# 30stomercury/whisper-char-alignment

Hardware: AMD Instinct MI355X
Metric: utterances/sec (whisper-medium, 10s audio, char align) at 1/2/4/8 MI355X (higher is better)
Workload: dtype f16x2 (hi + lo operand pairs on the f16 MFMA pipe: fp32-equivalent operands, fp32 accumulate)

## Files before the change

### whisper-char-alignment_amd/csrc/engine.hip

```cpp
#include <hip/hip_runtime.h>
#include <dlfcn.h>
#include <rccl/rccl.h>

#include <chrono>
#include <cmath>
#include <cstdarg>
#include <cstdio>
#include <cstdlib>
#include <cstring>
#include <deque>
#include <map>
#include <set>
#include <string>
#include <vector>

#include "../../include/wca.h"
#include "kernels.h"

using namespace wca;

namespace {

thread_local std::string g_err;

// ... 2877 lines not shown

int wca_test_gemm(wca_engine* e, const void* a, const void* w, const float* bias, void* c, int M, int N, int K, int gelu, int out_mode) {
  if (!e) return fail(WCA_ERR_INVALID, "null engine");
  HIPCHK(hipSetDevice(e->device));
  GemmArgs g{};
  g.A = (const half_t*)a;
  g.lda = K;
  g.W = (const half_t*)w;
  g.ldw = K;
  g.bias = bias;
  g.C = c;
  g.ldc = N;
  g.M = M;
  g.N = N;
  g.K = K;
  g.gelu = gelu;
  g.out_mode = out_mode & 0xff;
  if (g.out_mode == 4) {
    g.ldc = 2 * N;
    g.c_lo = N;
  }
  g.force_tile = (out_mode >> 8) & 0xfff;
  g.supertile = out_mode >> 20;
  g.sk_part = e->sk_big[0];
  g.sk_bytes = e->sk_big_bytes;
  HIPCHK(launch_gemm(g, e->stream));
  return WCA_OK;
}

int wca_test_gemm_pairs(wca_engine* e, const void* a2, const void* w, const float* bias, void* c, int M, int N, int K, int gelu, int out_mode) {
  if (!e || !a2 || !w || !c) return fail(WCA_ERR_INVALID, "null argument");
  HIPCHK(hipSetDevice(e->device));
  const int om = out_mode & 0xff;
  if (!gemm_splitw_supported(M, N, K, 2 * K, om)) return fail(WCA_ERR_INVALID, "the pair-operand kernel does not take M=%d N=%d K=%d out_mode %d", M, N, K, om);
  GemmArgs g{};
  g.A = (const half_t*)a2;
  g.lda = 2 * K;
  g.a_lo = K;
  g.W = (const half_t*)w;
  g.ldw = K;
  g.bias = bias;
  g.C = c;
  g.ldc = N;
  g.M = M;
  g.N = N;
  g.K = K;
  g.gelu = gelu;
  g.out_mode = om;
  if (om == 4) {
    g.ldc = 2 * N;
    g.c_lo = N;
  }
  g.force_tile = (out_mode >> 8) & 0xfff;
  g.site = 1;
  HIPCHK(launch_gemm(g, e->stream));
  return WCA_OK;
}

int wca_test_gemm_ln(wca_engine* e, const void* a, const void* w, const float* bias, float* x, const float* gamma, const float* beta,
                     void* xn, int M, int N, int K, int site) {
  if (!e || !a || !w || !x || !gamma || !beta || !xn) return fail(WCA_ERR_INVALID, "null argument");
  HIPCHK(hipSetDevice(e->device));
  if (!gemm_ln_supported(M, N, K, e->n_cu)) return fail(WCA_ERR_INVALID, "residual + LayerNorm epilogue not available for M=%d N=%d K=%d", M, N, K);
  const size_t mpad = align_up((size_t)M, 256);
  HIPCHK(e->tmp0.ensure(sizeof(unsigned long long) * (size_t)(N / 256) * mpad));
  HIPCHK(e->tmp1.ensure(sizeof(unsigned) * (mpad / 256 + 16)));
  HIPCHK(hipMemsetAsync(e->err_dev, 0, sizeof(int), e->stream));
// ... 236 lines not shown
```

### whisper-char-alignment_amd/csrc/gemm.hip

```cpp
#include <atomic>

#include "gemm_epilogue.h"
#include <cstdlib>
#include "kernels.h"
#include "wca_common.h"

namespace wca {

namespace {

constexpr int BM = 128, BN = 128, BK = 64;
constexpr int TILE_ELEMS = 128 * 64;

struct RowPtrs {
  const half_t* p[4];
};

__device__ __forceinline__ half8 ldfrag(const half_t* tile, int r, int c) {
  return *reinterpret_cast<const half8*>(tile + r * 64 + ((c ^ swz128(r)) << 3));
}

template <int OUT_MODE, bool GELU, int MT>
__device__ __forceinline__ void epilogue(const GemmArgs& a, f32x4 (&acc)[MT][4], int mbase, int nb, int fr) {
  float bv[16];
// ... 318 lines not shown
      for (int mt = 0; mt < 4; ++mt)
#pragma unroll
        for (int nt = 0; nt < 4; ++nt)
          acc[mt][nt] = __builtin_amdgcn_mfma_f32_16x16x32_f16(wf[ks][nt], xf[ks][mt], acc[mt][nt], 0, 0, 0);
    __builtin_amdgcn_s_setprio(0);

    half8 xg[2][4];
#pragma unroll
    for (int ks = 0; ks < 2; ++ks)
#pragma unroll
      for (int t = 0; t < 4; ++t) xg[ks][t] = ldfrag(At, xrow[4 + t], ks * 4 + fg);
    asm volatile("s_waitcnt lgkmcnt(0)" ::: "memory");
    __builtin_amdgcn_s_barrier();
    asm volatile("" ::: "memory");
    if (kt + 2 < nk) stage(cur, (kt + 2) * BK);
    __builtin_amdgcn_s_setprio(1);
#pragma unroll
    for (int ks = 0; ks < 2; ++ks)
#pragma unroll
      for (int mt = 0; mt < 4; ++mt)
#pragma unroll
        for (int nt = 0; nt < 4; ++nt)
          acc[4 + mt][nt] = __builtin_amdgcn_mfma_f32_16x16x32_f16(wf[ks][nt], xg[ks][mt], acc[4 + mt][nt], 0, 0, 0);
    __builtin_amdgcn_s_setprio(0);
  }

  epilogue<OUT_MODE, GELU, 8>(a, acc, m0 + wr * 128, n0 + wc * 64 + fg * 16, fr);
}

template <int V>
struct GemmIntC {
  static constexpr int value = V;
};

template <int OUT_MODE, bool GELU, int SITE, int SPLITW_MODE = 0>
__global__ __launch_bounds__(512) void gemm256p_f16_kernel(GemmArgs a) {
  constexpr bool SPLITW = SPLITW_MODE != 0;
  constexpr bool RING3 = SPLITW_MODE == 2;
  extern __shared__ __attribute__((aligned(16))) char smem[];
  half_t* lds = reinterpret_cast<half_t*>(smem);
  constexpr int TILE256 = 256 * 64;
  float* bias_lds = reinterpret_cast<float*>(smem + 4 * TILE256 * sizeof(half_t));
  float* gamma_lds = bias_lds + 512;
  float* beta_lds = gamma_lds + 512;
  float* ln_lds = beta_lds + 512;
  const int tid = threadIdx.x;
  const int lane = tid & 63;
  const int wave = __builtin_amdgcn_readfirstlane(tid >> 6);
  const int wr = wave >> 2, wc = wave & 3;

  const int ntn = (a.N + 255) / 256;
  const int ntm = (a.M + 255) / 256;
  const int nwg = ntm * ntn;
  const int G = gridDim.x;

  const __amdgpu_buffer_rsrc_t ra = __builtin_amdgcn_make_buffer_rsrc(const_cast<half_t*>(a.A), 0, (int)a.a_bytes, 0x00020000);
  const __amdgpu_buffer_rsrc_t rw = __builtin_amdgcn_make_buffer_rsrc(const_cast<half_t*>(a.W), 0, (int)a.w_bytes, 0x00020000);
  const __amdgpu_buffer_rsrc_t rb = __builtin_amdgcn_make_buffer_rsrc(const_cast<float*>(a.bias), 0, a.bias != nullptr ? a.N * 4 : 0, 0x00020000);
  const __amdgpu_buffer_rsrc_t rg = __builtin_amdgcn_make_buffer_rsrc(const_cast<float*>(a.ln_gamma), 0, OUT_MODE == 3 ? a.N * 4 : 0, 0x00020000);
  const __amdgpu_buffer_rsrc_t rbeta = __builtin_amdgcn_make_buffer_rsrc(const_cast<float*>(a.ln_beta), 0, OUT_MODE == 3 ? a.N * 4 : 0, 0x00020000);
  const int l8 = lane >> 3;
  const int rho = wave * 8 + l8;
  const int c0 = (lane & 7) ^ ((rho >> 1) & 7);
  const int nt_r = rho >> 4, i_r = rho & 15;
  const int wsrc_row = (OUT_MODE == 0 || OUT_MODE == 3 || OUT_MODE == 4) ? ((nt_r >> 1) * 32 + (i_r >> 2) * 8 + (nt_r & 1) * 4 + (i_r & 3)) : rho;
  const unsigned va = (unsigned)(rho * a.lda + c0 * 8) * 2u;
// ... 17 lines not shown
  auto stage_bias = [&](int par, int ncol0) {
    if (wave < 4) {
      __builtin_amdgcn_raw_ptr_buffer_load_lds(rb, (WCA_LDS void*)(bias_lds + par * 256 + wave * 64), 4, (ncol0 + wave * 64 + lane) * 4, 0, 0, 0);
      if (OUT_MODE == 3) {
        __builtin_amdgcn_raw_ptr_buffer_load_lds(rg, (WCA_LDS void*)(gamma_lds + par * 256 + wave * 64), 4, (ncol0 + wave * 64 + lane) * 4, 0, 0, 0);
        __builtin_amdgcn_raw_ptr_buffer_load_lds(rbeta, (WCA_LDS void*)(beta_lds + par * 256 + wave * 64), 4, (ncol0 + wave * 64 + lane) * 4, 0, 0, 0);
      }
    }
  };
  constexpr int RING3_A_REQS_IN_FLIGHT = 4;
  static_assert(RING3_A_REQS_IN_FLIGHT * 64 == 256, "one request per 64-row block of the 256-row A tile");

  const int fr = lane & 15, fg = lane >> 4;
  const int pos0 = fg ^ ((fr >> 1) & 7);
  const int xb0 = (wr * 128 + fr) * 64 + pos0 * 8, xb1 = (wr * 128 + fr) * 64 + (pos0 ^ 4) * 8;
  const int wb0 = (wc * 64 + fr) * 64 + pos0 * 8, wb1 = (wc * 64 + fr) * 64 + (pos0 ^ 4) * 8;

#define WCA_LOAD_HALF(AT, WT, XB, WB, WF, XF)                                                      \
  do {                                                                                             \
    _Pragma("unroll") for (int t = 0; t < 4; ++t) WF[t] = *reinterpret_cast<const half8*>((WT) + (WB) + t * 1024); \
    _Pragma("unroll") for (int t = 0; t < 8; ++t) XF[t] = *reinterpret_cast<const half8*>((AT) + (XB) + t * 1024); \
  } while (0)

  const int nk = SPLITW ? 2 * (a.K / BK) : a.K / BK;
  auto a_koff = [&](int s_) -> unsigned {
    return SPLITW ? (unsigned)(((s_ & 1) * (int)a.a_lo + (s_ >> 1) * BK) * 2) : (unsigned)(s_ * (BK * 2));
  };
  auto w_koff = [&](int s_) -> unsigned {
    return SPLITW ? (unsigned)((s_ >> 1) * (BK * 2)) : (unsigned)(s_ * (BK * 2));
  };
  int v = blockIdx.x;
  int id = xcd_remap(v, nwg);
  const int SM = a.supertile > 0 ? a.supertile : 1;
  auto tile_of = [&](int t, int& tm, int& tn) {
    const int per = SM * ntn;
    const int st = t / per, r = t - st * per;
    const int rows = (ntm - st * SM) < SM ? (ntm - st * SM) : SM;
    tn = r / rows;
    tm = st * SM + (r - tn * rows);
  };
  const int spx = G >> 3;
  const int PR = spx / ntn;
  const int lab = blockIdx.x & 7, slot = blockIdx.x >> 3;
  const int pq = ntm >> 3, prm = ntm & 7;
  const int lab_panels = pq + (lab < prm ? 1 : 0), lab_base = lab * pq + (lab < prm ? lab : prm);
  auto tile_of_round = [&](int round, int& tm, int& tn) -> bool {
    tn = slot / PR;
    const int pi = round * PR + (slot - tn * PR);
    tm = lab_base + pi;
    return tn < ntn && pi < lab_panels;
  };
  int tm_, tn_;
  int round = 0;
  if (OUT_MODE == 3) {
    if (!tile_of_round(0, tm_, tn_)) return;
  } else {
    tile_of(id, tm_, tn_);
  }
  int m0 = tm_ * 256, n0 = tn_ * 256;
  unsigned ta = (unsigned)m0 * a.lda * 2u, tw = (unsigned)n0 * a.ldw * 2u;

  f32x4 acc[8][4];
#pragma unroll
  for (int i = 0; i < 8; ++i)
#pragma unroll
    for (int j = 0; j < 4; ++j) acc[i][j] = f32x4{0.f, 0.f, 0.f, 0.f};
  half8 w0[4], x0[8], w1[4], x1[8];
  int par = 0;
  stage_bias(0, n0);
#pragma unroll
  for (int g = 0; g < 8; ++g) stage_one(0, 0, ta, tw, g);
  if (nk > 1) {
#pragma unroll
// ... 99 lines not shown

    {
      int fr_e = fr, fg_e = fg;
      asm volatile("" : "+v"(fr_e), "+v"(fg_e));
      typedef __attribute__((address_space(4))) GemmArgs KernArgs;
      const KernArgs* ap = (const KernArgs*)__builtin_amdgcn_kernarg_segment_ptr();
      asm volatile("" : "+s"(ap));
      if constexpr (OUT_MODE == 3)
        epilogue_ln<KernArgs>(*ap, acc, m0, m0 >> 8, n0 >> 8, ntn, wr, wc, fr_e, fg_e, bias_lds + par * 256 + wc * 64, gamma_lds + par * 256,
                              beta_lds + par * 256, ln_lds);
      else
        epilogue_wide<OUT_MODE, GELU, KernArgs>(*ap, acc, m0 + wr * 128, n0 + wc * 64, fr_e, fg_e, bias_lds + par * 256 + wc * 64);
    }
    if (!has_next) break;
    par ^= 1;
    stage_bias(par, n0n);
    v = vn;
    id = idn;
    ++round;
    m0 = m0n;
    n0 = n0n;
    ta = tan;
    tw = twn;
#pragma unroll
    for (int i = 0; i < 8; ++i)
#pragma unroll
      for (int j = 0; j < 4; ++j) acc[i][j] = f32x4{0.f, 0.f, 0.f, 0.f};
    WCA_LOAD_HALF(a_slot(RING3 ? ring_a : 0), w_slot(0), xb0, wb0, w0, x0);
  }
#undef WCA_LOAD_HALF
}


template <int OUT_MODE, bool GELU>
__global__ __launch_bounds__(256) void gemm_skinny_f16_kernel(GemmArgs a) {
  __shared__ float red[4][4][4][64];
  const int tid = threadIdx.x;
  const int lane = tid & 63;
  const int wave = __builtin_amdgcn_readfirstlane(tid >> 6);
  const int fr = lane & 15, fg = lane >> 4;
  const int n0 = blockIdx.x * 16;
  const int kq = a.K >> 2;
  const int kbeg = wave * kq;
  int nrow = n0 + fr;
  nrow = nrow < a.N ? nrow : a.N - 1;
  const half_t* wp = a.W + (long)nrow * a.ldw + kbeg + fg * 8;
  const half_t* xp[4];
#pragma unroll
  for (int mt = 0; mt < 4; ++mt) {
    int m = mt * 16 + fr;
    m = m < a.M ? m : a.M - 1;
    xp[mt] = a.A + (long)m * a.lda + kbeg + fg * 8;
  }
  f32x4 acc[4];
#pragma unroll
  for (int mt = 0; mt < 4; ++mt) acc[mt] = f32x4{0.f, 0.f, 0.f, 0.f};
  half8 wf[2][4], xf[2][4][4];
  auto load_chunk = [&](int buf, int k) {
#pragma unroll
    for (int u = 0; u < 4; ++u) {
      wf[buf][u] = *reinterpret_cast<const half8*>(wp + k + u * 32);
#pragma unroll
      for (int mt = 0; mt < 4; ++mt) xf[buf][u][mt] = *reinterpret_cast<const half8*>(xp[mt] + k + u * 32);
    }
  };
  auto mul_chunk = [&](int buf) {
// ... 37 lines not shown
    half_t* cp = reinterpret_cast<half_t*>(a.C) + coff + nb;
    if (nb + 4 <= a.N && (reinterpret_cast<uintptr_t>(cp) & 7) == 0) {
      half4 o;
#pragma unroll
      for (int r = 0; r < 4; ++r) o[r] = (half_t)v[r];
      *reinterpret_cast<half4*>(cp) = o;
    } else {
#pragma unroll
      for (int r = 0; r < 4; ++r)
        if (nb + r < a.N) cp[r] = (half_t)v[r];
    }
  } else {
    float* cp = reinterpret_cast<float*>(a.C) + coff + nb;
#pragma unroll
    for (int r = 0; r < 4; ++r)
      if (nb + r < a.N) cp[r] = (OUT_MODE == 2) ? cp[r] + v[r] : v[r];
  }
}

}

bool gemm_ln_supported(int M, int N, int K, int n_cu) {
  if (N % 256 != 0 || N > 2048 || K % 128 != 0 || M < 1) return false;
  const long tiles = (long)((M + 255) / 256) * (N / 256);
  if (tiles < 192) return false;
  return (n_cu >> 3) >= N / 256;
}

bool gemm_splitw_supported(int M, int N, int K, int lda, int out_mode) {
  if (M < 1 || N < 1 || K < 128 || (K % 128) != 0) return false;
  if (out_mode != 0 && out_mode != 1 && out_mode != 2 && out_mode != 4) return false;
  const long tiles256 = (long)((M + 255) / 256) * ((N + 255) / 256);
  if (tiles256 < 192) return false;
  const size_t a_need = ((size_t)(M - 1) * lda + 2 * (size_t)K) * sizeof(half_t), w_need = ((size_t)(N - 1) * K + K) * sizeof(half_t);
  return a_need < 0x7fffffffull && w_need < 0x7fffffffull;
}

hipError_t launch_gemm(const GemmArgs& a_in, hipStream_t s) {
  GemmArgs a = a_in;
  if (a.M <= 0 || a.N <= 0) return hipSuccess;
  if (a.K <= 0 || (a.K % BK) != 0) return hipErrorInvalidValue;
  if ((a.lda % 8) != 0 || (a.ldw % 8) != 0) return hipErrorInvalidValue;
  if (a.out_mode == 4 && (a.c_lo <= 0 || (a.c_lo & 7))) return hipErrorInvalidValue;
  if (a.addend != nullptr && (a.out_mode == 2 || a.out_mode == 3 || a.a_lo > 0)) return hipErrorInvalidValue;
  if ((a.force_tile == 64 || a.force_tile == 0) && a.M <= 64 && (a.K % 512) == 0 && a.a_rows_per_batch == 0 && a.pos == nullptr && a.addend == nullptr && a.out_mode != 4 && a.a_lo <= 0) {
    const dim3 sgrid((unsigned)((a.N + 15) / 16)), sblock(256);
#define WCA_LAUNCH_SK(OM, G) hipLaunchKernelGGL((gemm_skinny_f16_kernel<OM, G>), sgrid, sblock, 0, s, a)
    if (a.out_mode == 0) {
      if (a.gelu) WCA_LAUNCH_SK(0, true); else WCA_LAUNCH_SK(0, false);
    } else if (a.out_mode == 1) {
      if (a.gelu) WCA_LAUNCH_SK(1, true); else WCA_LAUNCH_SK(1, false);
    } else if (a.out_mode == 2 && !a.gelu) {
      WCA_LAUNCH_SK(2, false);
    } else {
      return hipErrorInvalidValue;
    }
#undef WCA_LAUNCH_SK
    return hipGetLastError();
  }
  if (a.force_tile == 64) return hipErrorInvalidValue;
  const long tiles256 = (long)((a.M + 255) / 256) * ((a.N + 255) / 256);
  const bool splitw = a.a_lo > 0;
  if (splitw && (a.force_tile == 64 || a.force_tile == 128 || a.force_tile == 256 || a.a_rows_per_batch != 0 ||
                 !gemm_splitw_supported(a.M, a.N, a.K, a.lda, a.out_mode) || (a.a_lo & 7) != 0))
    return hipErrorInvalidValue;
  const size_t a_need = ((size_t)(a.M - 1) * a.lda + (splitw ? (size_t)a.a_lo : 0) + a.K) * sizeof(half_t), w_need = ((size_t)(a.N - 1) * a.ldw + a.K) * sizeof(half_t);
  const bool can_buf = a.a_rows_per_batch == 0 && a_need < 0x7fffffffull && w_need < 0x7fffffffull;
  if (a.a_bytes == 0) a.a_bytes = (unsigned)a_need;
  if (a.w_bytes == 0) a.w_bytes = (unsigned)w_need;
  int dev = 0;
  {
    hipError_t e = hipGetDevice(&dev);
    if (e != hipSuccess) return e;
  }
  static std::atomic<int> n_cu_cache[32] = {};
  int n_cu = n_cu_cache[dev & 31].load(std::memory_order_relaxed);
  if (n_cu == 0) {
    hipError_t e = hipDeviceGetAttribute(&n_cu, hipDeviceAttributeMultiprocessorCount, dev);
    if (e != hipSuccess) return e;
    n_cu_cache[dev & 31].store(n_cu, std::memory_order_relaxed);
  }
  if (a.cu_limit > 0 && a.cu_limit < n_cu) n_cu = a.cu_limit;
  const int ring = splitw ? (debug_switch(DBG_GEMM_RING) == 1 ? 1 : 2) : 0;
  const bool want_big = (a.force_tile == 256 || a.force_tile == 257 || a.force_tile == 258) || (a.force_tile == 0 && tiles256 >= 192);
  const bool pipelined = want_big && can_buf && a.force_tile != 256 && a.addend == nullptr;
  const bool big = want_big;
  dim3 grid, block;
  size_t shmem;
  int splitk = 1;
  if (big) {
    grid = dim3((unsigned)tiles256);
    block = dim3(512);
    shmem = 2 * 2 * 256 * 64 * sizeof(half_t);
    if (pipelined) {
      shmem += 2 * 256 * sizeof(float);
      const int nk = (splitw ? 2 : 1) * (a.K / BK);
      if (a.force_tile != 258 && nk >= 2 && (nk & 1) == 0 && tiles256 > n_cu) grid = dim3((unsigned)n_cu);
      if (a.supertile <= 0) a.supertile = ((splitw ? 2 : 1) * a.K <= 2048 && (a.N + 255) / 256 <= 32) ? 8 : 1;
    }
  } else {
    const int ntn = (a.N + BN - 1) / BN, ntm = (a.M + BM - 1) / BM;
    grid = dim3(ntn * ntm);
    block = dim3(256);
    shmem = 2 * 2 * TILE_ELEMS * sizeof(half_t);
    splitk = 1;
    if (a.out_mode == 2 && !a.gelu && a.sk_part != nullptr && a.pos == nullptr && a.c_rows_per_batch == 0 && (a.N % 4) == 0 && (a.ldc % 4) == 0 &&
        ntn * ntm <= n_cu / 2 && a.K >= 2048) {
      for (int sk = 4; sk >= 2; --sk)
        if (a.K % (sk * BK) == 0 && (size_t)sk * a.M * a.N * sizeof(float) <= a.sk_bytes) {
          splitk = sk;
          break;
        }
    }
    grid.y = (unsigned)splitk;
  }
#define WCA_LAUNCH_K(...)                                                                         \
  do {                                                                                            \
    static std::atomic<unsigned> attr_mask{0};                                                    \
    if (!(attr_mask.load(std::memory_order_acquire) & (1u << (dev & 31)))) {                      \
      hipError_t e = hipFuncSetAttribute(reinterpret_cast<const void*>(__VA_ARGS__),              \
                                         hipFuncAttributeMaxDynamicSharedMemorySize, (int)shmem); \
      if (e != hipSuccess) return e;                                                              \
      attr_mask.fetch_or(1u << (dev & 31), std::memory_order_release);                            \
    }                                                                                             \
    hipLaunchKernelGGL((__VA_ARGS__), grid, block, shmem, s, a);                                  \
  } while (0)
#define WCA_LAUNCH_S(OM, G, S)                            \
  do {                                                    \
    if (pipelined && splitw && ring == 1) { if ((S) == 4) WCA_LAUNCH_K(gemm256p_f16_kernel<OM, G, 4, 1>); else WCA_LAUNCH_K(gemm256p_f16_kernel<OM, G, 1, 1>); } \
    else if (pipelined && splitw) { if ((S) == 4) WCA_LAUNCH_K(gemm256p_f16_kernel<OM, G, 4, 2>); else if ((S) == 3) WCA_LAUNCH_K(gemm256p_f16_kernel<OM, G, 3, 2>); else if ((S) == 2) WCA_LAUNCH_K(gemm256p_f16_kernel<OM, G, 2, 2>); else WCA_LAUNCH_K(gemm256p_f16_kernel<OM, G, 1, 2>); } \
    else if (pipelined) WCA_LAUNCH_K(gemm256p_f16_kernel<OM, G, S>); \
    else if (big) WCA_LAUNCH_K(gemm256_f16_kernel<OM, G, S>);  \
    else WCA_LAUNCH_K(gemm_f16_kernel<OM, G, S>);         \
  } while (0)
#define WCA_LAUNCH(OM, G)                     \
  do {                                        \
    switch (a.site) {                         \
      case 1: WCA_LAUNCH_S(OM, G, 1); break;  \
      case 2: WCA_LAUNCH_S(OM, G, 2); break;  \
      case 3: WCA_LAUNCH_S(OM, G, 3); break;  \
      case 4: WCA_LAUNCH_S(OM, G, 4); break;  \
      default: WCA_LAUNCH_S(OM, G, 0); break; \
    }                                         \
  } while (0)
  if (a.out_mode == 3) {
    if (!gemm_ln_supported(a.M, a.N, a.K, n_cu) || a.gelu || !pipelined || a.force_tile == 258 || a.pos != nullptr || a.c_rows_per_batch != 0 || !a.ln_gamma ||
        !a.ln_beta || !a.ln_out || !a.ln_stats || !a.ln_cnt || (a.ldc & 3) || (a.ln_ld & 7))
      return hipErrorInvalidValue;
    const size_t cnt_bytes = (((size_t)((a.M + 255) / 256) * sizeof(unsigned)) + 15) / 16 * 16;
    hipError_t e = hipMemsetAsync(a.ln_cnt, 0, cnt_bytes, s);
    if (e != hipSuccess) return e;
    shmem += (2 * 512 + 2560) * sizeof(float);
    grid = dim3((unsigned)(n_cu & ~7));
    switch (a.site) {
      case 4: WCA_LAUNCH_K(gemm256p_f16_kernel<3, false, 4>); break;
      default: WCA_LAUNCH_K(gemm256p_f16_kernel<3, false, 1>); break;
    }
  } else if (a.out_mode == 0) {
    if (a.gelu) WCA_LAUNCH(0, true); else WCA_LAUNCH(0, false);
  } else if (a.out_mode == 1) {
    if (a.gelu) WCA_LAUNCH(1, true); else WCA_LAUNCH(1, false);
  } else if (a.out_mode == 2) {
// ... 24 lines not shown
```

### whisper-char-alignment_amd/csrc/gemm_epilogue.h

```cpp
#pragma once
#include "kernels.h"
#include "wca_common.h"

namespace wca {

template <int OUT_MODE, bool GELU, typename ArgsT>
__device__ __forceinline__ void epilogue_wide(const ArgsT& a, f32x4 (&acc)[8][4], int mbase, int nbase, int fr, int fg, const float* bias_l) {
  int col[4];
#pragma unroll
  for (int nt = 0; nt < 4; ++nt) col[nt] = (OUT_MODE == 0 || OUT_MODE == 4) ? ((nt >> 1) * 32 + fg * 8 + (nt & 1) * 4) : (nt * 16 + fg * 4);
  float bv[16];
#pragma unroll
  for (int nt = 0; nt < 4; ++nt) {
    const f32x4 b4 = *reinterpret_cast<const f32x4*>(bias_l + col[nt]);
#pragma unroll
    for (int r = 0; r < 4; ++r) bv[nt * 4 + r] = b4[r];
  }
  const bool full_n = (nbase + 64 <= a.N);
  if (OUT_MODE == 2) {
    float* cbase = reinterpret_cast<float*>(a.C) + nbase;
    if (full_n && a.pos == nullptr && (a.ldc & 3) == 0 && (a.c_batch_stride & 3) == 0 && ((reinterpret_cast<uintptr_t>(cbase + fg * 4) & 15) == 0)) {
#pragma unroll
      for (int mt = 0; mt < 8; ++mt)
#pragma unroll
// ... 98 lines not shown
      } else {
#pragma unroll
        for (int nt = 0; nt < 4; ++nt)
#pragma unroll
          for (int r = 0; r < 4; ++r)
            if (nbase + col[nt] + r < a.N) {
              if (OUT_MODE == 4) {
                const HalfPair pr = split_pair(v[nt * 4 + r]);
                cp[col[nt] + r] = pr.hi;
                cp[a.c_lo + col[nt] + r] = pr.lo;
              } else {
                cp[col[nt] + r] = (half_t)v[nt * 4 + r];
              }
            }
      }
    } else {
      float* cp = reinterpret_cast<float*>(a.C) + coff + nbase;
      if (full_n && ((reinterpret_cast<uintptr_t>(cp + fg * 4) & 15) == 0)) {
#pragma unroll
        for (int nt = 0; nt < 4; ++nt) {
          f32x4* c4 = reinterpret_cast<f32x4*>(cp + col[nt]);
          f32x4 o = f32x4{v[nt * 4 + 0], v[nt * 4 + 1], v[nt * 4 + 2], v[nt * 4 + 3]};
          if (OUT_MODE == 2) o += *c4;
          *c4 = o;
        }
      } else {
#pragma unroll
        for (int nt = 0; nt < 4; ++nt)
#pragma unroll
          for (int r = 0; r < 4; ++r)
            if (nbase + col[nt] + r < a.N) cp[col[nt] + r] = (OUT_MODE == 2) ? cp[col[nt] + r] + v[nt * 4 + r] : v[nt * 4 + r];
      }
    }
  }
}

__device__ __forceinline__ float xor16_sum(float v) {
  const unsigned u = __float_as_uint(v);
  auto r = __builtin_amdgcn_permlane16_swap(u, u, false, false);
  return __uint_as_float(r[0]) + __uint_as_float(r[1]);
}
__device__ __forceinline__ float xor32_sum(float v) {
  const unsigned u = __float_as_uint(v);
  auto r = __builtin_amdgcn_permlane32_swap(u, u, false, false);
  return __uint_as_float(r[0]) + __uint_as_float(r[1]);
}
__device__ __forceinline__ void chan_merge(float& mean_a, float& m2_a, float na, float mean_b, float m2_b, float nb) {
  const float dlt = mean_b - mean_a, nt = na + nb;
  mean_a += dlt * (nb / nt);
  m2_a += m2_b + dlt * dlt * (na * nb / nt);
}

typedef __attribute__((address_space(1))) unsigned long long gu64_t;
typedef __attribute__((address_space(1))) unsigned gu32_t;

template <typename ArgsT>
__device__ __forceinline__ void epilogue_ln(const ArgsT& a, f32x4 (&acc)[8][4], int m0, int tm, int tn, int ntn, int wr, int wc, int fr, int fg,
                                            const float* bias_l, const float* gamma_l, const float* beta_l, float* ln_lds) {
  const int tid = threadIdx.x;
  const int mbase = m0 + wr * 128, nbase = tn * 256 + wc * 64;
  int col[4];
#pragma unroll
  for (int nt = 0; nt < 4; ++nt) col[nt] = (nt >> 1) * 32 + fg * 8 + (nt & 1) * 4;
  {
    float bv[16];
#pragma unroll
// ... 146 lines not shown
```

### whisper-char-alignment_amd/csrc/kernels.h

```cpp
#pragma once
#include <hip/hip_runtime.h>
#include <stdint.h>

namespace wca {

typedef _Float16 half_t;

enum { DBG_ATTN_SPLIT_VARIANT = 0, DBG_HEAD_STATS_GENERAL, DBG_FAIL_PRECISION_ALLOC, DBG_ATTN_SPLIT_DROP, DBG_GEMM_RING, DBG_SWITCH_COUNT };
int debug_switch(int id);
int set_debug_switch(const char* name, int value);

struct GemmArgs {
  const half_t* A;
  long a_lo;
  int lda;
  int a_rows_per_batch;
  long a_batch_stride;
  const half_t* W;
  int ldw;
  const float* bias;
  void* C;
  int ldc;
  int c_rows_per_batch;
  long c_batch_stride;
// ... 7 lines not shown
  int out_mode;
  unsigned a_bytes, w_bytes;
  int force_tile;
  const float* ln_gamma;
  const float* ln_beta;
  half_t* ln_out;
  int ln_ld;
  float ln_eps;
  unsigned long long* ln_stats;
  unsigned* ln_cnt;
  int* ln_err;
  int site;
  int supertile;
  int cu_limit;
  const float* A32;
  int lda32;
  half_t* kv_k;
  half_t* kv_v;
  long kv_bs;
  int kv_t, kv_d;
  size_t sk_bytes;
  float* sk_part;
  unsigned* sk_cnt;
  int splitk;
  int groups;
};
hipError_t launch_gemm(const GemmArgs& a, hipStream_t s);
hipError_t launch_gemm_rows(const GemmArgs& a, hipStream_t s);
bool gemm_rows_supported(int M, int N, int K, bool layernorm_a);
int gemm_rows_pick_splitk(int K);
size_t gemm_rows_workspace_bytes(int M, int N, int splitk);
bool gemm_ln_supported(int M, int N, int K, int n_cu);
bool gemm_splitw_supported(int M, int N, int K, int lda, int out_mode);

struct AttnArgs {
  const half_t* Q; long q_bs; int q_rs;
  const half_t* K; long k_bs; int k_rs;
  const half_t* V; long v_bs; int v_rs;
  half_t* O; long o_bs; int o_rs;
  float* cap;
  long cap_bs; long cap_hs; int cap_ld;
  int cap_cols;
  int nq, nk, H, B;
  float scale;
  int causal;
  int variant;
  int split;
  long q_lo, k_lo, v_lo, o_lo;
};
hipError_t launch_attention(const AttnArgs& a, hipStream_t s);
hipError_t launch_attention_split(const AttnArgs& a, hipStream_t s);

hipError_t launch_layernorm_f16(const float* x, const float* gamma, const float* beta, half_t* out,
                                int rows, int d, float eps, hipStream_t s, int ld_out = 0, long lo_off = 0);
hipError_t launch_embed(const int64_t* tokens, const half_t* tok_emb, const float* pos_emb, float* x,
                        int B, int n, int d, int n_vocab, int* err, hipStream_t s, const half_t* tok_emb_lo = nullptr);
hipError_t launch_fill_f16(half_t* p, size_t n, float v, hipStream_t s);

hipError_t launch_embed_step(const int* tokens, int T_max, int t, const half_t* tok_emb, const float* pos_emb, float* x, int B, int d,
                             int n_vocab, hipStream_t s);
hipError_t launch_kv_append(const half_t* qkv, half_t* kc, half_t* vc, int B, int T_max, int t, int d, hipStream_t s);
hipError_t launch_embed_prefix(const int* tokens, int T_max, int n, const half_t* tok_emb, const float* pos_emb, float* x, int B, int d,
                               int n_vocab, hipStream_t s);
hipError_t launch_kv_scatter(const half_t* qkv, half_t* kc, half_t* vc, int B, int n, int T_max, int d, hipStream_t s);
hipError_t launch_gather_rows(const float* x, float* out, int B, int n, int p0, int p1, int d, hipStream_t s);
struct DecodeSelectArgs {
// ... 114 lines not shown
```

Before: 336.8.

## Add persistent 256x128 pair-operand GEMM with epilogue deferred into next tile's mainloop

Adds a persistent 256x128-tile GEMM kernel for hi/lo pair operands. It keeps a three-deep A ring in LDS and overlaps the previous tile's bias/GELU/split/store epilogue with the first four k-steps of the next tile. By default it is selected for the K=1024 sites 1 and 3 in out modes 2 and 4, and a force_tile value of 259 also selects it. The aim is to hide epilogue and store latency and to get more tiles from narrower N tiles. The cost is extra registers for the deferred accumulators, which may lower occupancy, plus more dispatch complexity.

After: 313.6. 0.931x the previous value.

```diff
diff --git a/whisper-char-alignment_amd/csrc/engine.hip b/whisper-char-alignment_amd/csrc/engine.hip
--- a/whisper-char-alignment_amd/csrc/engine.hip
+++ b/whisper-char-alignment_amd/csrc/engine.hip
@@ -2933,7 +2933,8 @@
   if (!e || !a2 || !w || !c) return fail(WCA_ERR_INVALID, "null argument");
   HIPCHK(hipSetDevice(e->device));
   const int om = out_mode & 0xff;
-  if (!gemm_splitw_supported(M, N, K, 2 * K, om)) return fail(WCA_ERR_INVALID, "the pair-operand kernel does not take M=%d N=%d K=%d out_mode %d", M, N, K, om);
+  const bool ok = ((out_mode >> 8) & 0xfff) == 259 ? gemm_deferred_supported(M, N, K, 2 * K, om) : gemm_splitw_supported(M, N, K, 2 * K, om);
+  if (!ok) return fail(WCA_ERR_INVALID, "the pair-operand kernel does not take M=%d N=%d K=%d out_mode %d", M, N, K, om);
   GemmArgs g{};
   g.A = (const half_t*)a2;
   g.lda = 2 * K;
diff --git a/whisper-char-alignment_amd/csrc/gemm.hip b/whisper-char-alignment_amd/csrc/gemm.hip
--- a/whisper-char-alignment_amd/csrc/gemm.hip
+++ b/whisper-char-alignment_amd/csrc/gemm.hip
@@ -374,6 +374,14 @@
 struct GemmIntC {
   static constexpr int value = V;
 };
+
+__device__ __forceinline__ void supertile_of(int t, int ntm, int ntn, int SM, int& tm, int& tn) {
+  const int per = SM * ntn;
+  const int st = t / per, r = t - st * per;
+  const int rows = (ntm - st * SM) < SM ? (ntm - st * SM) : SM;
+  tn = r / rows;
+  tm = st * SM + (r - tn * rows);
+}
 
 template <int OUT_MODE, bool GELU, int SITE, int SPLITW_MODE = 0>
 __global__ __launch_bounds__(512) void gemm256p_f16_kernel(GemmArgs a) {
@@ -457,13 +465,7 @@
   int v = blockIdx.x;
   int id = xcd_remap(v, nwg);
   const int SM = a.supertile > 0 ? a.supertile : 1;
-  auto tile_of = [&](int t, int& tm, int& tn) {
-    const int per = SM * ntn;
-    const int st = t / per, r = t - st * per;
-    const int rows = (ntm - st * SM) < SM ? (ntm - st * SM) : SM;
-    tn = r / rows;
-    tm = st * SM + (r - tn * rows);
-  };
+  auto tile_of = [&](int t, int& tm, int& tn) { supertile_of(t, ntm, ntn, SM, tm, tn); };
   const int spx = G >> 3;
   const int PR = spx / ntn;
   const int lab = blockIdx.x & 7, slot = blockIdx.x >> 3;
@@ -629,6 +631,242 @@
 }
 
 
+template <int OUT_MODE, bool GELU, int SITE>
+__global__ __launch_bounds__(512) void gemm256x128d_f16_kernel(GemmArgs a) {
+  extern __shared__ __attribute__((aligned(16))) char smem[];
+  half_t* lds = reinterpret_cast<half_t*>(smem);
+  constexpr int TILE_A = 256 * 64;
+  half_t* const w_lds = lds + 3 * TILE_A;
+  float* bias_lds = reinterpret_cast<float*>(smem + (3 * TILE_A + 128 * 64) * sizeof(half_t));
+  const int tid = threadIdx.x;
+  const int lane = tid & 63;
+  const int wave = __builtin_amdgcn_readfirstlane(tid >> 6);
+  const int wr = wave >> 1, wc = wave & 1;
+
+  const int ntn = (a.N + 127) / 128;
+  const int ntm = (a.M + 255) / 256;
+  const int nwg = ntm * ntn;
+  const int G = gridDim.x;
+
+  const __amdgpu_buffer_rsrc_t ra = __builtin_amdgcn_make_buffer_rsrc(const_cast<half_t*>(a.A), 0, (int)a.a_bytes, 0x00020000);
+  const __amdgpu_buffer_rsrc_t rw = __builtin_amdgcn_make_buffer_rsrc(const_cast<half_t*>(a.W), 0, (int)a.w_bytes, 0x00020000);
+  const __amdgpu_buffer_rsrc_t rb = __builtin_amdgcn_make_buffer_rsrc(const_cast<float*>(a.bias), 0, a.bias != nullptr ? a.N * 4 : 0, 0x00020000);
+  const int l8 = lane >> 3;
+  const int rho = wave * 8 + l8;
+  const int c0 = (lane & 7) ^ ((rho >> 1) & 7);
+  const int nt_r = rho >> 4, i_r = rho & 15;
+  const int wsrc_row = (OUT_MODE == 0 || OUT_MODE == 4) ? ((nt_r >> 1) * 32 + (i_r >> 2) * 8 + (nt_r & 1) * 4 + (i_r & 3)) : rho;
+  const unsigned va = (unsigned)(rho * a.lda + c0 * 8) * 2u;
+  const unsigned vw = (unsigned)(wsrc_row * a.ldw + c0 * 8) * 2u;
+  const unsigned sa64 = 64u * a.lda * 2u, sw64 = 64u * a.ldw * 2u;
+  auto a_slot = [&](int buf) -> half_t* { return lds + buf * TILE_A; };
+  auto stage_a = [&](int buf, unsigned ta_k, int i) {
+    unsigned so = ta_k + i * sa64;
+    asm volatile("" : "+s"(so));
+    __builtin_amdgcn_raw_ptr_buffer_load_lds(ra, (WCA_LDS void*)(a_slot(buf) + (i * 64 + wave * 8) * 64), 16, (int)(va + so), 0, 0, 0);
+  };
+  auto stage_w = [&](unsigned tw_k, int i) {
+    unsigned so = tw_k + i * sw64;
+    asm volatile("" : "+s"(so));
+    __builtin_amdgcn_raw_ptr_buffer_load_lds(rw, (WCA_LDS void*)(w_lds + (i * 64 + wave * 8) * 64), 16, (int)(vw + so), 0, 0, 0);
+  };
+  auto stage_bias = [&](int par, int ncol0) {
+    if (wave < 2) __builtin_amdgcn_raw_ptr_buffer_load_lds(rb, (WCA_LDS void*)(bias_lds + par * 128 + wave * 64), 4, (ncol0 + wave * 64 + lane) * 4, 0, 0, 0);
+  };
+  constexpr int RING3_A_REQS_IN_FLIGHT = 4;
+  constexpr int DRAIN_STORES = drain_stores<OUT_MODE>();
+
+  const int fr = lane & 15, fg = lane >> 4;
+  const int pos0 = fg ^ ((fr >> 1) & 7);
+  const int xb0 = (wr * 64 + fr) * 64 + pos0 * 8, xb1 = (wr * 64 + fr) * 64 + (pos0 ^ 4) * 8;
+  const int wb0 = (wc * 64 + fr) * 64 + pos0 * 8, wb1 = (wc * 64 + fr) * 64 + (pos0 ^ 4) * 8;
+
+  const int nk = 2 * (a.K / BK);
+  auto a_koff = [&](int s_) -> unsigned { return (unsigned)(((s_ & 1) * (int)a.a_lo + (s_ >> 1) * BK) * 2); };
+  auto w_koff = [&](int s_) -> unsigned { return (unsigned)((s_ >> 1) * (BK * 2)); };
+
+  int v = blockIdx.x;
+  int id = xcd_remap(v, nwg);
+  const int SM = a.supertile > 0 ? a.supertile : 1;
+  int tm_, tn_;
+  supertile_of(id, ntm, ntn, SM, tm_, tn_);
+  int m0 = tm_ * 256, n0 = tn_ * 128;
+  unsigned ta = (unsigned)m0 * a.lda * 2u, tw = (unsigned)n0 * a.ldw * 2u;
+
+  f32x4 acc[4][4], dr[4][4];
+#pragma unroll
+  for (int i = 0; i < 4; ++i)
+#pragma unroll
+    for (int j = 0; j < 4; ++j) {
+      acc[i][j] = f32x4{0.f, 0.f, 0.f, 0.f};
+      dr[i][j] = f32x4{0.f, 0.f, 0.f, 0.f};
+    }
+  half8 w0[4], x0[4], w1[4], x1[4];
+  DrainRegs dregs;
+  char WCA_GLOBAL* d_crow = nullptr;
+  long d_step = 0, d_lo = 0;
+  int d_rows = 0;
+  const float* d_bias = bias_lds;
+  bool d_whole = false;
+  bool pending = false;
+  typedef __attribute__((address_space(4))) GemmArgs KernArgs;
+  auto kernargs = [&]() -> const KernArgs* {
+    const KernArgs* ap = (const KernArgs*)__builtin_amdgcn_kernarg_segment_ptr();
+    asm volatile("" : "+s"(ap));
+    return ap;
+  };
+  auto drain_setup = [&](int m0_, int n0_, int par_) {
+    const KernArgs* ap = kernargs();
+    constexpr int ES = (OUT_MODE == 0 || OUT_MODE == 4) ? 2 : 4;
+    constexpr int LW = (OUT_MODE == 0 || OUT_MODE == 4) ? 8 : 4;
+    int fr_e = fr, fg_e = fg;
+    asm volatile("" : "+v"(fr_e), "+v"(fg_e));
+    d_bias = bias_lds + par_ * 128 + wc * 64;
+    d_whole = m0_ + 256 <= ap->M;
+    d_rows = ap->M - (m0_ + wr * 64 + fr_e);
+    d_crow = (char WCA_GLOBAL*)(ap->C) + ((long)(m0_ + wr * 64 + fr_e) * ap->ldc + n0_ + wc * 64 + fg_e * LW) * ES;
+    d_step = 16L * ap->ldc * ES;
+    d_lo = OUT_MODE == 4 ? ap->c_lo * 2 : 0;
+  };
+
+  int par = 0;
+  stage_bias(0, n0);
+#pragma unroll
+  for (int i = 0; i < 4; ++i) stage_a(0, ta, i);
+#pragma unroll
+  for (int i = 0; i < 2; ++i) stage_w(tw, i);
+#pragma unroll
+  for (int i = 0; i < 4; ++i) stage_a(1, ta + a_koff(1), i);
+  asm volatile("s_waitcnt vmcnt(4)" ::: "memory");
+  __builtin_amdgcn_s_barrier();
+  asm volatile("" ::: "memory");
+#pragma unroll
+  for (int t = 0; t < 4; ++t) w0[t] = *reinterpret_cast<const half8*>(w_lds + wb0 + t * 1024);
+#pragma unroll
+  for (int t = 0; t < 4; ++t) x0[t] = *reinterpret_cast<const half8*>(a_slot(0) + xb0 + t * 1024);
+  int ring_a = 0;
+
+  for (;;) {
+    const int vn = v + G;
+    const bool has_next = vn < nwg;
+    const int idn = has_next ? xcd_remap(vn, nwg) : id;
+    int tmn_, tnn_;
+    supertile_of(idn, ntm, ntn, SM, tmn_, tnn_);
+    const int m0n = tmn_ * 256, n0n = tnn_ * 128;
+    const unsigned tan = (unsigned)m0n * a.lda * 2u, twn = (unsigned)n0n * a.ldw * 2u;
+    auto kstep = [&](auto piece_c, const int kt) {
+      constexpr int P = decltype(piece_c)::value;
+      const bool last = kt + 1 == nk;
+      const int cur = ring_a;
+      const int nxt = cur == 2 ? 0 : cur + 1;
+      const int prv = cur == 0 ? 2 : cur - 1;
+      const bool W_FRESH = (kt & 1) == 0;
+      const half_t* At = a_slot(cur);
+      const bool in_tile2 = kt + 2 < nk;
+      const bool more1 = !last || has_next, more2 = in_tile2 || has_next;
+      const unsigned ka = (in_tile2 ? ta + a_koff(kt + 2) : tan + a_koff(kt + 2 - nk));
+      const unsigned kw = (in_tile2 ? tw + w_koff(kt + 2) : twn + w_koff(kt + 2 - nk));
+      const bool exact = P >= 0 && d_whole;
+#pragma unroll
+      for (int g = 0; g < 4; ++g) {
+        __builtin_amdgcn_s_setprio(1);
+#pragma unroll
+        for (int nt = 0; nt < 4; ++nt) acc[g][nt] = __builtin_amdgcn_mfma_f32_16x16x32_f16(w0[nt], x0[g], acc[g][nt], 0, 0, 0);
+        __builtin_amdgcn_s_setprio(0);
+        __builtin_amdgcn_sched_barrier(0);
+        if (g < 2) {
+          if (W_FRESH) {
+            w1[2 * g] = *reinterpret_cast<const half8*>(w_lds + wb1 + (2 * g) * 1024);
+            w1[2 * g + 1] = *reinterpret_cast<const half8*>(w_lds + wb1 + (2 * g + 1) * 1024);
+          }
+        } else {
+          x1[2 * (g - 2)] = *reinterpret_cast<const half8*>(At + xb1 + (2 * (g - 2)) * 1024);
+          x1[2 * (g - 2) + 1] = *reinterpret_cast<const half8*>(At + xb1 + (2 * (g - 2) + 1) * 1024);
+        }
+        if (more2) stage_a(prv, ka, g);
+        if (P >= 0) {
+          constexpr int PP = P >= 0 ? P : 0;
+          drain_quarter<OUT_MODE, GELU>(dregs, g, dr[PP][g], d_bias, fg);
+          if (g == 3 && PP * 16 < d_rows) drain_store<OUT_MODE>(dregs, d_crow + PP * d_step, d_lo);
+        }
+        __builtin_amdgcn_sched_barrier(0);
+      }
+      if (more2) {
+        if (exact) asm volatile("s_waitcnt vmcnt(%0) lgkmcnt(0)" ::"i"(RING3_A_REQS_IN_FLIGHT + DRAIN_STORES) : "memory");
+        else asm volatile("s_waitcnt vmcnt(%0) lgkmcnt(0)" ::"i"(RING3_A_REQS_IN_FLIGHT) : "memory");
+      } else {
+        if (exact) asm volatile("s_waitcnt vmcnt(%0) lgkmcnt(0)" ::"i"(DRAIN_STORES) : "memory");
+        else asm volatile("s_waitcnt vmcnt(0) lgkmcnt(0)" ::: "memory");
+      }
+      __builtin_amdgcn_s_barrier();
+      asm volatile("" ::: "memory");
+      const half_t* An = a_slot(nxt);
+#pragma unroll
+      for (int g = 0; g < 4; ++g) {
+        __builtin_amdgcn_s_setprio(1);
+#pragma unroll
+        for (int nt = 0; nt < 4; ++nt) acc[g][nt] = __builtin_amdgcn_mfma_f32_16x16x32_f16(w1[nt], x1[g], acc[g][nt], 0, 0, 0);
+        __builtin_amdgcn_s_setprio(0);
+        __builtin_amdgcn_sched_barrier(0);
+        if (W_FRESH && (g & 1) == 1 && more2) stage_w(kw, g >> 1);
+        if (more1) {
+          if (g < 2) {
+            if (!W_FRESH) {
+              w0[2 * g] = *reinterpret_cast<const half8*>(w_lds + wb0 + (2 * g) * 1024);
+              w0[2 * g + 1] = *reinterpret_cast<const half8*>(w_lds + wb0 + (2 * g + 1) * 1024);
+            }
+          } else {
+            x0[2 * (g - 2)] = *reinterpret_cast<const half8*>(An + xb0 + (2 * (g - 2)) * 1024);
+            x0[2 * (g - 2) + 1] = *reinterpret_cast<const half8*>(An + xb0 + (2 * (g - 2) + 1) * 1024);
+          }
+        }
+        if (OUT_MODE == 2 && g == 0 && P >= 0 && P < 3 && (P + 1) * 16 < d_rows) drain_preload(dregs, d_crow + (P + 1) * d_step);
+        __builtin_amdgcn_sched_barrier(0);
+      }
+      ring_a = nxt;
+    };
+    int kt0 = 0;
+    if (pending) {
+      kstep(GemmIntC<0>{}, 0);
+      kstep(GemmIntC<1>{}, 1);
+      kstep(GemmIntC<2>{}, 2);
+      kstep(GemmIntC<3>{}, 3);
+      kt0 = 4;
+    }
+    for (int kt = kt0; kt < nk; ++kt) kstep(GemmIntC<-1>{}, kt);
+    if (!has_next) break;
+    drain_setup(m0, n0, par);
+    if (OUT_MODE == 2 && 0 < d_rows) drain_preload(dregs, d_crow);
+#pragma unroll
+    for (int i = 0; i < 4; ++i)
+#pragma unroll
+      for (int j = 0; j < 4; ++j) {
+        dr[i][j] = acc[i][j];
+        acc[i][j] = f32x4{0.f, 0.f, 0.f, 0.f};
+      }
+    pending = true;
+    par ^= 1;
+    stage_bias(par, n0n);
+    v = vn;
+    id = idn;
+    m0 = m0n;
+    n0 = n0n;
+    ta = tan;
+    tw = twn;
+  }
+  drain_setup(m0, n0, par);
+#pragma unroll
+  for (int p = 0; p < 4; ++p) {
+    if (p * 16 < d_rows) {
+      if (OUT_MODE == 2) drain_preload(dregs, d_crow + p * d_step);
+#pragma unroll
+      for (int g = 0; g < 4; ++g) drain_quarter<OUT_MODE, GELU>(dregs, g, acc[p][g], d_bias, fg);
+      drain_store<OUT_MODE>(dregs, d_crow + p * d_step, d_lo);
+    }
+  }
+}
+
+
 template <int OUT_MODE, bool GELU>
 __global__ __launch_bounds__(256) void gemm_skinny_f16_kernel(GemmArgs a) {
   __shared__ float red[4][4][4][64];
@@ -732,6 +970,31 @@
   if (out_mode != 0 && out_mode != 1 && out_mode != 2 && out_mode != 4) return false;
   const long tiles256 = (long)((M + 255) / 256) * ((N + 255) / 256);
   if (tiles256 < 192) return false;
+  const size_t a_need = ((size_t)(M - 1) * lda + 2 * (size_t)K) * sizeof(half_t), w_need = ((size_t)(N - 1) * K + K) * sizeof(half_t);
+  return a_need < 0x7fffffffull && w_need < 0x7fffffffull;
+}
+
+namespace {
+bool gemm_deferred_args(const GemmArgs& a) {
+  const int lw = (a.out_mode == 0 || a.out_mode == 4) ? 8 : 4;
+  return gemm_deferred_supported(a.M, a.N, a.K, a.lda, a.out_mode) && a.pos == nullptr && a.c_rows_per_batch == 0 && (a.ldc % lw) == 0 &&
+         (reinterpret_cast<uintptr_t>(a.C) & 15) == 0 && !(a.gelu && a.out_mode != 4);
+}
+bool gemm_deferred_site(const GemmArgs& a) {
+  if (a.K != 1024 || !gemm_deferred_args(a)) return false;
+  if (a.site == 1 && a.out_mode == 4) return true;
+  if (a.site == 1 && a.out_mode == 2) return true;
+  if (a.site == 3 && a.out_mode == 4) return true;
+  return false;
+}
+}
+
+bool gemm_deferred_supported(int M, int N, int K, int lda, int out_mode) {
+  if (M < 1 || N < 1 || K < 128 || (K % 128) != 0) return false;
+  if ((N % 128) != 0) return false;
+  if (out_mode != 0 && out_mode != 1 && out_mode != 2 && out_mode != 4) return false;
+  const long tiles = (long)((M + 255) / 256) * ((N + 127) / 128);
+  if (tiles < 192) return false;
   const size_t a_need = ((size_t)(M - 1) * lda + 2 * (size_t)K) * sizeof(half_t), w_need = ((size_t)(N - 1) * K + K) * sizeof(half_t);
   return a_need < 0x7fffffffull && w_need < 0x7fffffffull;
 }
@@ -761,8 +1024,11 @@
   if (a.force_tile == 64) return hipErrorInvalidValue;
   const long tiles256 = (long)((a.M + 255) / 256) * ((a.N + 255) / 256);
   const bool splitw = a.a_lo > 0;
-  if (splitw && (a.force_tile == 64 || a.force_tile == 128 || a.force_tile == 256 || a.a_rows_per_batch != 0 ||
-                 !gemm_splitw_supported(a.M, a.N, a.K, a.lda, a.out_mode) || (a.a_lo & 7) != 0))
+  if (a.force_tile == 259 && (!splitw || a.a_rows_per_batch != 0 || a.addend != nullptr || (a.a_lo & 7) != 0 || !gemm_deferred_args(a)))
+    return hipErrorInvalidValue;
+  if (splitw && a.force_tile != 259 &&
+      (a.force_tile == 64 || a.force_tile == 128 || a.force_tile == 256 || a.a_rows_per_batch != 0 ||
+       !gemm_splitw_supported(a.M, a.N, a.K, a.lda, a.out_mode) || (a.a_lo & 7) != 0))
     return hipErrorInvalidValue;
   const size_t a_need = ((size_t)(a.M - 1) * a.lda + (splitw ? (size_t)a.a_lo : 0) + a.K) * sizeof(half_t), w_need = ((size_t)(a.N - 1) * a.ldw + a.K) * sizeof(half_t);
   const bool can_buf = a.a_rows_per_batch == 0 && a_need < 0x7fffffffull && w_need < 0x7fffffffull;
@@ -782,13 +1048,20 @@
   }
   if (a.cu_limit > 0 && a.cu_limit < n_cu) n_cu = a.cu_limit;
   const int ring = splitw ? (debug_switch(DBG_GEMM_RING) == 1 ? 1 : 2) : 0;
-  const bool want_big = (a.force_tile == 256 || a.force_tile == 257 || a.force_tile == 258) || (a.force_tile == 0 && tiles256 >= 192);
+  const bool want_big = (a.force_tile == 256 || a.force_tile == 257 || a.force_tile == 258 || a.force_tile == 259) || (a.force_tile == 0 && tiles256 >= 192);
   const bool pipelined = want_big && can_buf && a.force_tile != 256 && a.addend == nullptr;
   const bool big = want_big;
+  const bool deferred = pipelined && splitw && ring == 2 && a.out_mode != 3 && (a.force_tile == 259 || (a.force_tile == 0 && gemm_deferred_site(a)));
   dim3 grid, block;
   size_t shmem;
   int splitk = 1;
-  if (big) {
+  if (deferred) {
+    const long tiles = (long)((a.M + 255) / 256) * ((a.N + 127) / 128);
+    grid = dim3((unsigned)(tiles > n_cu ? n_cu : tiles));
+    block = dim3(512);
+    shmem = (3 * 256 * 64 + 128 * 64) * sizeof(half_t) + 2 * 128 * sizeof(float);
+    if (a.supertile <= 0) a.supertile = (2 * a.K <= 2048 && (a.N + 255) / 256 <= 32) ? 8 : 1;
+  } else if (big) {
     grid = dim3((unsigned)tiles256);
     block = dim3(512);
     shmem = 2 * 2 * 256 * 64 * sizeof(half_t);
@@ -827,7 +1100,9 @@
   } while (0)
 #define WCA_LAUNCH_S(OM, G, S)                            \
   do {                                                    \
-    if (pipelined && splitw && ring == 1) { if ((S) == 4) WCA_LAUNCH_K(gemm256p_f16_kernel<OM, G, 4, 1>); else WCA_LAUNCH_K(gemm256p_f16_kernel<OM, G, 1, 1>); } \
+    if (deferred && (G) && (OM) != 4) return hipErrorInvalidValue; \
+    else if (deferred) { if ((S) == 3) WCA_LAUNCH_K(gemm256x128d_f16_kernel<OM, (OM) == 4 && (G), 3>); else WCA_LAUNCH_K(gemm256x128d_f16_kernel<OM, (OM) == 4 && (G), 1>); } \
+    else if (pipelined && splitw && ring == 1) { if ((S) == 4) WCA_LAUNCH_K(gemm256p_f16_kernel<OM, G, 4, 1>); else WCA_LAUNCH_K(gemm256p_f16_kernel<OM, G, 1, 1>); } \
     else if (pipelined && splitw) { if ((S) == 4) WCA_LAUNCH_K(gemm256p_f16_kernel<OM, G, 4, 2>); else if ((S) == 3) WCA_LAUNCH_K(gemm256p_f16_kernel<OM, G, 3, 2>); else if ((S) == 2) WCA_LAUNCH_K(gemm256p_f16_kernel<OM, G, 2, 2>); else WCA_LAUNCH_K(gemm256p_f16_kernel<OM, G, 1, 2>); } \
     else if (pipelined) WCA_LAUNCH_K(gemm256p_f16_kernel<OM, G, S>); \
     else if (big) WCA_LAUNCH_K(gemm256_f16_kernel<OM, G, S>);  \
diff --git a/whisper-char-alignment_amd/csrc/gemm_epilogue.h b/whisper-char-alignment_amd/csrc/gemm_epilogue.h
--- a/whisper-char-alignment_amd/csrc/gemm_epilogue.h
+++ b/whisper-char-alignment_amd/csrc/gemm_epilogue.h
@@ -154,6 +154,72 @@
             if (nbase + col[nt] + r < a.N) cp[col[nt] + r] = (OUT_MODE == 2) ? cp[col[nt] + r] + v[nt * 4 + r] : v[nt * 4 + r];
       }
     }
+  }
+}
+
+struct DrainRegs {
+  f32x4 f[4];
+  half4 hi[4];
+  half4 lo[4];
+};
+template <int OUT_MODE>
+__device__ __forceinline__ int drain_col(int nt, int fg) {
+  return (OUT_MODE == 0 || OUT_MODE == 4) ? ((nt >> 1) * 32 + fg * 8 + (nt & 1) * 4) : (nt * 16 + fg * 4);
+}
+template <int OUT_MODE>
+constexpr int drain_stores() { return OUT_MODE == 0 ? 2 : 4; }
+
+__device__ __forceinline__ void drain_preload(DrainRegs& d, const char WCA_GLOBAL* crow) {
+  const f32x4 WCA_GLOBAL* cp = reinterpret_cast<const f32x4 WCA_GLOBAL*>(crow);
+#pragma unroll
+  for (int nt = 0; nt < 4; ++nt) d.f[nt] = cp[nt * 4];
+}
+template <int OUT_MODE, bool GELU>
+__device__ __forceinline__ void drain_quarter(DrainRegs& d, int nt, const f32x4& accq, const float* bias_l, int fg) {
+  const f32x4 b4 = *reinterpret_cast<const f32x4*>(bias_l + drain_col<OUT_MODE>(nt, fg));
+  float v[4];
+#pragma unroll
+  for (int r = 0; r < 4; ++r) v[r] = accq[r] + b4[r];
+  if (GELU) {
+#pragma unroll
+    for (int j = 0; j < 4; j += 2) {
+      if (OUT_MODE == 4) {
+        const f32x2 g = gelu_erfc2(f32x2{v[j], v[j + 1]});
+        v[j] = g[0];
+        v[j + 1] = g[1];
+      } else {
+        v[j] = gelu_erf(v[j]);
+        v[j + 1] = gelu_erf(v[j + 1]);
+      }
+    }
+  }
+  if (OUT_MODE == 4) {
+    const Half2Pair p0 = split_pair2(v[0], v[1]), p1 = split_pair2(v[2], v[3]);
+    d.hi[nt] = half4{p0.hi[0], p0.hi[1], p1.hi[0], p1.hi[1]};
+    d.lo[nt] = half4{p0.lo[0], p0.lo[1], p1.lo[0], p1.lo[1]};
+  } else if (OUT_MODE == 0) {
+    d.hi[nt] = half4{(half_t)v[0], (half_t)v[1], (half_t)v[2], (half_t)v[3]};
+  } else {
+    f32x4 o = f32x4{v[0], v[1], v[2], v[3]};
+    if (OUT_MODE == 2) o += d.f[nt];
+    d.f[nt] = o;
+  }
+}
+template <int OUT_MODE>
+__device__ __forceinline__ void drain_store(const DrainRegs& d, char WCA_GLOBAL* crow, long c_lo_bytes) {
+  if (OUT_MODE == 0 || OUT_MODE == 4) {
+#pragma unroll
+    for (int hh = 0; hh < 2; ++hh) {
+      const half4 a0 = d.hi[2 * hh], a1 = d.hi[2 * hh + 1];
+      *reinterpret_cast<half8 WCA_GLOBAL*>(crow + hh * 64) = half8{a0[0], a0[1], a0[2], a0[3], a1[0], a1[1], a1[2], a1[3]};
+      if (OUT_MODE == 4) {
+        const half4 l0 = d.lo[2 * hh], l1 = d.lo[2 * hh + 1];
+        *reinterpret_cast<half8 WCA_GLOBAL*>(crow + c_lo_bytes + hh * 64) = half8{l0[0], l0[1], l0[2], l0[3], l1[0], l1[1], l1[2], l1[3]};
+      }
+    }
+  } else {
+#pragma unroll
+    for (int nt = 0; nt < 4; ++nt) *reinterpret_cast<f32x4 WCA_GLOBAL*>(crow + nt * 64) = d.f[nt];
   }
 }
 
diff --git a/whisper-char-alignment_amd/csrc/kernels.h b/whisper-char-alignment_amd/csrc/kernels.h
--- a/whisper-char-alignment_amd/csrc/kernels.h
+++ b/whisper-char-alignment_amd/csrc/kernels.h
@@ -63,6 +63,7 @@
 size_t gemm_rows_workspace_bytes(int M, int N, int splitk);
 bool gemm_ln_supported(int M, int N, int K, int n_cu);
 bool gemm_splitw_supported(int M, int N, int K, int lda, int out_mode);
+bool gemm_deferred_supported(int M, int N, int K, int lda, int out_mode);
 
 struct AttnArgs {
   const half_t* Q; long q_bs; int q_rs;
```
